# candrewlee14/zgml

Hardware: AMD Instinct MI355X
Metric: decode_tokens_per_sec (higher is better)
Workload: dtype f32; 1 GPU; SmolLM-135M Q4_0 greedy decode, batch 1, 1xMI355X (BASELINE configs[1]); weights=synthetic Q4_0 (int4 + f16 block scale / 32), tied f32 LM head, max_seq=2048, loop=device-resident (inputs in HBM), parallelism=none

## Files before the change

### zgml_amd/csrc/attention_decode.h

```cpp
#pragma once
#include "kernels.h"
#include "handoff_gen.h"
#include <hip/hip_fp16.h>
#include <math.h>

namespace zgml {
namespace {

typedef float f4v_t __attribute__((ext_vector_type(4)));
__device__ __forceinline__ float4 ldg4(const float* p) {
    const f4v_t v = *(const __attribute__((address_space(1))) f4v_t*)p;
    return make_float4(v.x, v.y, v.z, v.w);
}
__device__ __forceinline__ float ldg1(const float* p) { return *(const __attribute__((address_space(1))) float*)p; }
__device__ __forceinline__ uint32_t ldgu(const uint32_t* p) { return *(const __attribute__((address_space(1))) uint32_t*)p; }
__device__ __forceinline__ void stg4(float* p, float4 v) { *(__attribute__((address_space(1))) f4v_t*)p = f4v_t{v.x, v.y, v.z, v.w}; }
__device__ __forceinline__ void stg1(float* p, float v) { *(__attribute__((address_space(1))) float*)p = v; }
__device__ __forceinline__ void stgu(uint32_t* p, uint32_t v) { *(__attribute__((address_space(1))) uint32_t*)p = v; }

constexpr int kAttnBlock = 1024;
constexpr int kAttnUnroll = 4;

__device__ __forceinline__ float4 rope4(float4 own, float4 par, float4 c, float4 s, bool is_hi) {
    if (is_hi)
// ... 35 lines not shown
    if (LPK >= 2) v += __int_as_float(__builtin_amdgcn_mov_dpp(__float_as_int(v), 0xB1, 0xF, 0xF, true));
    if (LPK >= 4) v += __int_as_float(__builtin_amdgcn_mov_dpp(__float_as_int(v), 0x4E, 0xF, 0xF, true));
    if (LPK >= 8) v += __int_as_float(__builtin_amdgcn_mov_dpp(__float_as_int(v), 0x141, 0xF, 0xF, true));
    if (LPK >= 16) v += __int_as_float(__builtin_amdgcn_mov_dpp(__float_as_int(v), 0x140, 0xF, 0xF, true));
    if (LPK >= 32) v = xor16_sum(v);
    if (LPK >= 64) v = xor32_sum(v);
    return v;
}

struct SoftState {
    float m, l;
    float4 acc;
};
__device__ __forceinline__ void soft_merge(SoftState& s, float om, float ol, float4 oacc) {
    const float nm = fmaxf(s.m, om);
    const float a = s.m > -INFINITY ? expf(s.m - nm) : 0.0f, b = om > -INFINITY ? expf(om - nm) : 0.0f;
    s.l = s.l * a + ol * b;
    s.acc = make_float4(s.acc.x * a + oacc.x * b, s.acc.y * a + oacc.y * b, s.acc.z * a + oacc.z * b, s.acc.w * a + oacc.w * b);
    s.m = nm;
}

using gu64 = __attribute__((address_space(1))) unsigned long long;
using gu32 = __attribute__((address_space(1))) unsigned int;
__device__ __forceinline__ void split_put(float* p, float a, float b) {
    const unsigned long long v = (unsigned long long)__float_as_uint(a) | ((unsigned long long)__float_as_uint(b) << 32);
    __hip_atomic_store((gu64*)p, v, __ATOMIC_RELAXED, __HIP_MEMORY_SCOPE_AGENT);
}
__device__ __forceinline__ void split_get(const float* p, float& a, float& b) {
    const unsigned long long v = __hip_atomic_load((gu64*)p, __ATOMIC_RELAXED, __HIP_MEMORY_SCOPE_AGENT);
    a = __uint_as_float((uint32_t)v), b = __uint_as_float((uint32_t)(v >> 32));
}

template <int LPK>
__device__ __forceinline__ void slots_sum(SoftState& s) {
#pragma unroll
    for (int off = LPK; off < 16; off <<= 1) {
        s.l += __shfl_xor(s.l, off, 64);
        s.acc.x += __shfl_xor(s.acc.x, off, 64), s.acc.y += __shfl_xor(s.acc.y, off, 64);
        s.acc.z += __shfl_xor(s.acc.z, off, 64), s.acc.w += __shfl_xor(s.acc.w, off, 64);
    }
    if (LPK <= 16) s.l = xor16_sum(s.l), s.acc.x = xor16_sum(s.acc.x), s.acc.y = xor16_sum(s.acc.y), s.acc.z = xor16_sum(s.acc.z), s.acc.w = xor16_sum(s.acc.w);
    if (LPK <= 32) s.l = xor32_sum(s.l), s.acc.x = xor32_sum(s.acc.x), s.acc.y = xor32_sum(s.acc.y), s.acc.z = xor32_sum(s.acc.z), s.acc.w = xor32_sum(s.acc.w);
}
template <int LPK>
__device__ __forceinline__ void slots_merge(SoftState& s) {
    float M = s.m;
// ... 86 lines not shown
        __builtin_amdgcn_sched_barrier(0);
#endif
    }
}
template <int L, bool MAX>
__device__ __forceinline__ float slots_all(float v) {
    auto op = [](float a, float b) { return MAX ? fmaxf(a, b) : a + b; };
    if (L <= 1) v = op(v, __int_as_float(__builtin_amdgcn_mov_dpp(__float_as_int(v), 0x121, 0xF, 0xF, true)));
    if (L <= 2) v = op(v, __int_as_float(__builtin_amdgcn_mov_dpp(__float_as_int(v), 0x122, 0xF, 0xF, true)));
    if (L <= 4) v = op(v, __int_as_float(__builtin_amdgcn_mov_dpp(__float_as_int(v), 0x124, 0xF, 0xF, true)));
    if (L <= 8) v = op(v, __int_as_float(__builtin_amdgcn_mov_dpp(__float_as_int(v), 0x128, 0xF, 0xF, true)));
    if (L <= 16) v = MAX ? xor16_max(v) : xor16_sum(v);
    if (L <= 32) v = MAX ? xor32_max(v) : xor32_sum(v);
    return v;
}

struct DecodeHandoff {
    const unsigned long long* gran;
    uint32_t rel[3];
    uint32_t* gen;
    uint32_t n_heads;
    uint32_t* timeout;
    uint32_t poll_sleep;
};
__device__ __forceinline__ void handoff_idle(const DecodeHandoff* ho, uint32_t wg, uint32_t gen) { ho->gen[wg] = gen; }
__device__ __forceinline__ void handoff_idle(const CounterHandoff* ho, uint32_t wg, uint32_t) { for (int c = 0; c < 3; c++) ho->seen[3 * wg + c] += ho->need; }
__device__ __forceinline__ void handoff_done(const DecodeHandoff* ho, uint32_t wg, uint32_t gen, const uint32_t (&)[3]) { ho->gen[wg] = gen; }
__device__ __forceinline__ void handoff_done(const CounterHandoff* ho, uint32_t wg, uint32_t, const uint32_t (&t)[3]) { for (int c = 0; c < 3; c++) ho->seen[3 * wg + c] = t[c]; }
template <int LPK, bool KVQ, int BLOCK = kAttnBlock, typename HO = DecodeHandoff>
__device__ __forceinline__ void attention_decode_body(const AttnDecodeParams* __restrict__ params, float* split_buf, uint32_t* split_cnt,
                                                      uint32_t split_min_keys, const uint32_t hx, const uint32_t sp_in, const uint32_t n_sp, const HO* ho) {
    constexpr bool COUNTERS = std::is_same<HO, CounterHandoff>::value;
    constexpr int DH = 4 * LPK, HALF = DH / 2;
    constexpr bool Q16 = KVQ && ZGML_ATTN_KVQ16 != 0 && LPK >= 32;
    constexpr int LPKM = Q16 ? DH / 16 : LPK, KPW = 64 / LPKM, KPW4 = 64 / LPK, U = Q16 ? kAttnUnrollQ16 : kAttnUnroll;
    using Row = AttnRow<KVQ>;
    static_assert(sizeof(AttnDecodeParams) == 248, "the bulk fetch below covers exactly 62 dwords");
    AttnDecodeParams P;
    {
        typedef uint32_t u32x16_t __attribute__((ext_vector_type(16)));
        typedef uint32_t u32x8_t __attribute__((ext_vector_type(8)));
        typedef uint32_t u32x4_t __attribute__((ext_vector_type(4)));
        typedef uint32_t u32x2_t __attribute__((ext_vector_type(2)));
        u32x16_t ra, rb, rc;
        u32x8_t rd;
        u32x4_t re;
// ... 373 lines not shown
            ml[i] = *(const float2*)&part_ml[2 * wc];
            pa[i] = part_acc[wc * LPK + li];
        }
        M = fmaxf(M, __int_as_float(__builtin_amdgcn_mov_dpp(__float_as_int(M), 0xB1, 0xF, 0xF, true)));
        M = fmaxf(M, __int_as_float(__builtin_amdgcn_mov_dpp(__float_as_int(M), 0x4E, 0xF, 0xF, true)));
        M = fmaxf(M, __int_as_float(__builtin_amdgcn_mov_dpp(__float_as_int(M), 0x141, 0xF, 0xF, true)));
        M = fmaxf(M, __int_as_float(__builtin_amdgcn_mov_dpp(__float_as_int(M), 0x140, 0xF, 0xF, true)));
        M = __int_as_float(__builtin_amdgcn_readfirstlane(__float_as_int(M)));
        r = SoftState{M, 0.f, make_float4(0.f, 0.f, 0.f, 0.f)};
#pragma unroll
        for (int i = 0; i < NPS; i++) {
            const bool live = slot + i * KPW4 < NW && ml[i].x > -INFINITY;
            const float f = live ? expf(ml[i].x - M) : 0.0f;
            r.l += ml[i].y * f;
            r.acc.x += pa[i].x * f, r.acc.y += pa[i].y * f, r.acc.z += pa[i].z * f, r.acc.w += pa[i].w * f;
        }
        slots_sum<LPK>(r);
    } else {
        ATTN_STAMP(5);
        ATTN_STAMP(6);
    }
    {
        if (wait_qkv && lane == 0) handoff_done(ho, hx * n_sp + sp, gen, target);
        if (n_active > 1) {
            constexpr uint32_t REC = DH + 4;
            float* const head_buf = split_buf + (uint64_t)hx * n_sp * REC;
            float* const mine = head_buf + (uint64_t)sp * REC;
            if (lane < LPK) {
                if (lane == 0) split_put(mine, r.m, r.l);
                split_put(mine + 4 + 4 * lane, r.acc.x, r.acc.y);
                split_put(mine + 4 + 4 * lane + 2, r.acc.z, r.acc.w);
            }
            asm volatile("s_waitcnt vmcnt(0)" ::: "memory");
            uint32_t old = 0;
            if (lane == 0) old = __hip_atomic_fetch_add((gu32*)(split_cnt + hx), 1u, __ATOMIC_RELAXED, __HIP_MEMORY_SCOPE_AGENT);
            old = __shfl(old, 0, 64);
            if (old != n_active - 1) return;
            __builtin_amdgcn_fence(__ATOMIC_ACQUIRE, "wavefront");
            r = SoftState{-INFINITY, 0.f, make_float4(0.f, 0.f, 0.f, 0.f)};
            for (uint32_t c = slot; c < n_active; c += KPW4) {
                const float* rec = head_buf + (uint64_t)c * REC;
                float om, ol;
                float4 oa;
                split_get(rec, om, ol);
                split_get(rec + 4 + 4 * li, oa.x, oa.y);
                split_get(rec + 4 + 4 * li + 2, oa.z, oa.w);
// ... 28 lines not shown
```

### zgml_amd/csrc/kernels.h

```cpp
#pragma once

#include <hip/hip_runtime.h>
#include <stdint.h>
#include <stdlib.h>

#include "../../include/zgml_hip.h"
#include "sample.h"
#include "switches.h"

namespace zgml {

inline uint32_t device_cus() {
    static const uint32_t n = [] {
        int dev = 0, cus = 0;
        if (hipGetDevice(&dev) != hipSuccess || hipDeviceGetAttribute(&cus, hipDeviceAttributeMultiprocessorCount, dev) != hipSuccess || cus <= 0) cus = 256;
        return (uint32_t)cus;
    }();
    return n;
}

constexpr int kMaxFusedSteps = 8;

struct FusedStepDev {
    uint32_t op;
// ... 492 lines not shown
                  uint64_t* sc_bytes);
void launch_pack_qweight(hipStream_t s, const int8_t* raw_data, const float* raw_scales, const QWeightDev& out);
constexpr uint64_t kQmmScratchHead = 16384;
constexpr uint64_t kQmmCounterBytes = 4096;
uint64_t qmatmul_scratch_bytes(const QWeightDev& w, uint32_t M);
void launch_qmatmul(hipStream_t s, const QWeightDev& w, const QMatmulParams& p, float* scratch);
constexpr uint32_t kKonRowsMaxM = 8;
constexpr uint32_t kKonRowsRoutedM = 6;
bool launch_qmatvec_kon_rows(hipStream_t s, const QWeightDev& w, const QMatmulParams& p);
bool qmatmul_can_group(const QWeightDev& a, const QMatmulParams& pa, const QWeightDev& b, const QMatmulParams& pb);
uint32_t qmatmul_max_group();
void launch_qmatmul_group(hipStream_t s, const QWeightDev* w, const QMatmulParams* p, uint32_t n, float* scratch);
bool qmv_prenorm_ok(const QWeightDev& w, uint32_t K, uint64_t total_cols, uint32_t M);
bool qmv_pair_ok(const QWeightDev& w);
bool qmv_can_group(const QWeightDev& a, const QWeightDev& b);
uint32_t qmv_max_prologue_k(const QWeightDev& w);
void launch_qmatvec_fused(hipStream_t s, const QmvLaunch& L);
struct QkvHandoffBlock {
    unsigned long long* granules = nullptr;
    uint32_t *producer_gen = nullptr, *consumer_gen = nullptr;
    uint32_t* counters = nullptr;
    const uint32_t* idx = nullptr;
    uint32_t* seen = nullptr;
};
bool launch_qkv_attention(hipStream_t s, const QmvLaunch& L, const AttnDecodeParams* dev_params, uint32_t n_heads, uint32_t n_kv, uint32_t d_head,
                          const AttnSplit& sp, const QkvHandoffBlock& hb, uint32_t* timeout, bool kvq = false);
int qkv_attn_kon_census(hipStream_t s, uint32_t d_head, bool kvq, uint32_t grid);
int qkv_attn_kon_blocks_per_cu(uint32_t d_head, bool kvq);
void launch_synth_packed(hipStream_t s, const QWeightDev& w, uint32_t matrix_id);

struct KsVec {
    const float* base = nullptr;
    const float* parts = nullptr;
    uint32_t n_parts = 0;
    float* sum_dst = nullptr;
    float* add_dst = nullptr;
};
struct KsNormIn {
    KsVec x;
    const float* gamma = nullptr;
    float eps = 0.f;
    float* store_mid = nullptr;
    float* store_x = nullptr;
    uint32_t K = 0;
};
struct KsProjLaunch {
// ... 66 lines not shown
```

### zgml_amd/csrc/plan.hip

```cpp
#include "runtime_internal.h"

namespace {

float* buf_at(zgml_hip_program* p, uint16_t idx, uint64_t off) { return p->bufs[idx] + off; }

template <typename T>
const T* upload_params(zgml_hip_program* p, const std::vector<T>& v) {
    void* d = nullptr;
    if (hipMalloc(&d, v.size() * sizeof(T)) != hipSuccess) {
        p->ctx->fail("plan: parameter array allocation failed");
        return nullptr;
    }
    if (h2d_sync(p->ctx->stream, d, v.data(), v.size() * sizeof(T)) != hipSuccess) p->ctx->fail("plan: parameter array upload failed");
    p->param_blobs.push_back(d);
    return (const T*)d;
}

AttnSplit attn_split_for(zgml_hip_program* p, uint32_t n_heads, uint32_t d_head, uint32_t max_kv, int default_min_keys = 128) {
    const int want = sw().hip_attn_split;
    const int min_keys_env = sw().hip_attn_split_min_keys;
    AttnSplit sp;
    const int64_t min_keys = p->ctx->opt_attn_split_min_keys >= 0 ? p->ctx->opt_attn_split_min_keys : (min_keys_env >= 0 ? min_keys_env : default_min_keys);
    if (min_keys == 0 || want <= 1) return sp;
    sp.min_keys = (uint32_t)std::min<int64_t>(std::max<int64_t>(32, min_keys), 1 << 30);
// ... 501 lines not shown
}

void fuse_qkv_attention(zgml_hip_program* p) {
    if (!sw().hip_fuse_qkv_attn || p->ctx->fuse_qkv_off || !p->ctx->handoff_flag_dev) return;
    const uint64_t resident_cap = p->ctx->opt_fuse_resident_wgs >= 0 ? (uint64_t)p->ctx->opt_fuse_resident_wgs : (uint64_t)std::max(p->ctx->n_cu, 1);
    for (size_t i = 0; i + 1 < p->plan.size(); i++) {
        const auto qd = p->plan[i].qmv_desc;
        const auto ad = p->plan[i + 1].adec_desc;
        if (!qd || !ad) continue;
        const QmvLaunch& L = *qd;
        if (barrier_between_launches(p, i)) continue;
        const bool kon = L.parts[0].w.format == QW_Q4K && L.K > 2048;
        if (L.n_parts != 3 || (L.K > 2048 && !(kon && sw().hip_fuse_qkv_attn_kon)) || L.pro.kind == QMV_PRO_NONE || (ad->dh != 64 && ad->dh != 128) || L.trace) continue;
        if (kon && L.pro.kind != QMV_PRO_PRENORM) continue;
        const bool kvq = ad->kvq;
        bool ok = true;
        for (uint32_t t = 0; t < 3; t++) ok = ok && L.parts[t].n_epi == 0 && (L.parts[t].w.format == QW_Q4 || L.parts[t].w.format == QW_Q4K) && L.parts[t].w.scale_f16;
        const uint32_t nh = ad->nh, dh = ad->dh;
        ok = ok && (uint64_t)nh * dh == L.parts[0].w.N && L.parts[1].w.N == L.parts[2].w.N && L.parts[1].w.N % dh == 0;
        const uint32_t n_kv = ok ? (uint32_t)(L.parts[1].w.N / dh) : 0;
        ok = ok && n_kv != 0 && nh % n_kv == 0;
        std::vector<uint32_t> idx(3 * (size_t)nh);
        std::vector<char> head_seen(nh, 0);
        for (uint32_t r = 0; ok && r < nh; r++) {
            const AttnDecodeParams& a = ad->host[r];
            const ptrdiff_t qo = a.q_src - L.parts[0].dst, ko = a.k_src - L.parts[1].dst, vo = a.v_src - L.parts[2].dst;
            ok = qo >= 0 && qo % dh == 0 && (uint64_t)qo < (uint64_t)nh * dh && ko >= 0 && ko % dh == 0 && (uint64_t)ko < (uint64_t)n_kv * dh && vo == ko &&
                 a.kvq_block == (kvq ? 32u : 0u);
            if (!ok) break;
            const uint32_t h = (uint32_t)(qo / dh), kvh = (uint32_t)(ko / dh);
            ok = !head_seen[h] && kvh == h / (nh / n_kv);
            head_seen[h] = 1;
            idx[3 * r] = h, idx[3 * r + 1] = nh + kvh, idx[3 * r + 2] = nh + n_kv + kvh;
        }
        if (!ok) continue;
        uint32_t n_sp = ad->sp.splits ? ad->sp.splits : 1;
        uint64_t n_mv = 0;
        for (uint32_t t = 0; t < 3; t++) n_mv += L.parts[t].w.N / 16;
        uint64_t cap = resident_cap;
        if (kon && p->ctx->opt_fuse_resident_wgs < 0) {
            const int per_cu = qkv_attn_kon_blocks_per_cu(ad->dh, kvq);
            cap = per_cu > 0 ? (uint64_t)per_cu * (uint64_t)std::max(p->ctx->n_cu, 1) * (uint64_t)sw().hip_fuse_kon_cap_eighths / 8 : 0;
        }
        if (n_mv + nh > cap) continue;
        if (kon && p->ctx->opt_fuse_resident_wgs < 0 && (cap - n_mv) / nh < n_sp) continue;
        n_sp = (uint32_t)std::min<uint64_t>(n_sp, (cap - n_mv) / nh);
        for (uint32_t t = 0; kon && t < 3; t++) ok = ok && L.parts[t].w.format == QW_Q4K;
        if (!ok) continue;
        if (kon && p->ctx->opt_fuse_resident_wgs < 0) {
            const uint32_t grid = (uint32_t)(n_mv + (uint64_t)nh * n_sp);
            const uint64_t key = ((uint64_t)ad->dh << 40) | ((uint64_t)(kvq ? 1 : 0) << 32) | grid;
            auto it = p->ctx->census.find(key);
            if (it == p->ctx->census.end()) {
                const int r = sw().hip_fuse_census ? qkv_attn_kon_census(p->ctx->stream, ad->dh, kvq, grid) : -1;
                it = p->ctx->census.emplace(key, r).first;
                if (r == 0) fprintf(stderr, "[zgml_hip] the fused q/k/v + attention launch of %u workgroups is NOT co-resident on this device (census): two launches instead\n", grid);
            }
            if (it->second == 0) continue;
        }
        const size_t n_gran = ((size_t)nh + 2 * n_kv) * dh, n_cnt = 32 * ((size_t)nh + 2 * n_kv);
        const size_t bytes = kon ? (n_cnt + (size_t)nh * n_sp * 3 + 1 + idx.size()) * 4 : (n_gran * 8 + (n_mv + (size_t)nh * n_sp) * 4 + 15) / 16 * 16;
        void* block = nullptr;
        if (hipMalloc(&block, bytes) != hipSuccess) continue;
        if (memset_sync(p->ctx->stream, block, 0, bytes) != hipSuccess) {
            hipFree(block);
            continue;
        }
        p->fuse_owned.push_back(block);
        uint32_t* const timeout = p->ctx->handoff_flag_dev;
        QkvHandoffBlock hb;
        if (kon) {
            hb.counters = (uint32_t*)block, hb.seen = hb.counters + n_cnt;
            uint32_t* const idx_dev = hb.seen + (size_t)nh * n_sp * 3 + 1;
            if (h2d_sync(p->ctx->stream, idx_dev, idx.data(), idx.size() * 4) != hipSuccess) continue;
            hb.idx = idx_dev;
        } else {
            hb.granules = (unsigned long long*)block;
            hb.producer_gen = (uint32_t*)(hb.granules + n_gran), hb.consumer_gen = hb.producer_gen + n_mv;
        }
        const AttnDecodeParams* d = ad->dev;
        AttnSplit sp = ad->sp;
        sp.splits = n_sp;
        const uint32_t n_ops = p->plan[i].n_ops + p->plan[i + 1].n_ops, lo = std::min(p->plan[i].op_lo, p->plan[i + 1].op_lo),
                       hi = std::max(p->plan[i].op_hi, p->plan[i + 1].op_hi);
        Launch F{ZGML_DOP_QMATMUL, n_ops, lo, hi, [=](hipStream_t s) {
                     if (!launch_qkv_attention(s, L, d, nh, n_kv, dh, sp, hb, timeout, kvq)) {
                         launch_qmatvec_fused(s, L);
                         launch_attention_decode_batch(s, d, nh, dh, sp, kvq);
                     }
                 }};
        p->plan[i] = std::move(F);
        p->plan.erase(p->plan.begin() + (ptrdiff_t)i + 1);
    }
}

void fuse_ksplit(zgml_hip_program* p) {
    p->has_deferred = false;
    if (!p->ksplit || p->ksplit_off || !p->barriers.empty()) return;
    auto overlap = [](const float* a, size_t na, const float* b, size_t nb) { return a && b && a < b + nb && b < a + na; };
    auto residual_epi = [](const QmvPart& pt) {
        return pt.n_epi == 1 && pt.epi[0].op == ZGML_OP_ADD && pt.epi[0].operand && pt.epi[0].operand != pt.dst && pt.epi[0].store && pt.epi[0].store != pt.dst;
// ... 1121 lines not shown
```

### zgml_amd/csrc/qmatvec.hip

```cpp
#include "qmv_common.h"
#include "attention_decode.h"

#include <hip/hip_fp16.h>
#include <math.h>
#include <stdlib.h>
#include <string.h>

#include <type_traits>
#include <utility>

namespace zgml {

namespace {



struct QMVPartDev {
    const uint4* qs;
    const void* sc;
    float* out;
    uint32_t NB2;
    uint32_t block_begin;
    uint32_t out_rs;
    uint32_t n_epi;
// ... 110 lines not shown
                                             bool have_pre0 = false) {
    const float raw = v;
#pragma unroll
    for (uint32_t e = 0; e < (uint32_t)kMaxEpiSteps; e++) {
        if (e >= part.n_epi) break;
        const QmvEpiStep st = part.epi[e];
        if (st.op == ZGML_OP_ADD) {
            const float o = st.operand == out_row ? raw : (e == 0 && have_pre0 ? pre0 : st.operand[n]);
            v = st.swapped ? o + v : v + o;
        } else if (st.op == ZGML_OP_MUL) {
            const float o = st.operand == out_row ? raw : (e == 0 && have_pre0 ? pre0 : st.operand[n]);
            v = st.swapped ? o * v : v * o;
        } else {
            v = epi_unary(st.op, v);
        }
        if (st.store) st.store[n] = v;
    }
}

struct QmvPublish {
    unsigned long long* gran;
    uint32_t* gen;
    uint32_t drop;
};
struct QmvCountPublish {
    uint32_t* cnt;
    uint32_t base[3];
    uint32_t groups_shift;
    uint32_t drop;
};

struct KonTail {
    float post;
    bool norm;
    float eps;
    uint32_t K;
    float a_s, b_s;
    uint32_t k0, slice;
    bool has_pro;
    bool prenorm;
    float pp[4];
    bool inv_known = false;
    float inv_pre = 1.0f;
};
__device__ __forceinline__ float prenorm_factor(const float (&pp)[4], uint32_t K, float eps) {
    const float ss = rows_sum4(row16_sum((pp[0] + pp[1]) + (pp[2] + pp[3])));
    return 1.0f / sqrtf(ss / (float)K + eps);
}
__device__ __forceinline__ float kon_factor_and_slices(const KonTail& kt, const QMVArgs& a, const float* red, uint32_t n_waves, uint32_t lane) {
    const uint32_t col = lane & 15;
    float inv = 1.0f;
    if (kt.inv_known) {
        inv = kt.inv_pre;
    } else if (kt.prenorm) {
        float s4 = (kt.pp[0] + kt.pp[1]) + (kt.pp[2] + kt.pp[3]);
        for (uint32_t j = lane + 256; j < a.pro.n_ssq; j += 64) s4 += a.pro.ssq[j];
        const float ss = rows_sum4(row16_sum(s4));
        inv = 1.0f / sqrtf(ss / (float)kt.K + kt.eps);
    } else if (kt.norm) {
        const float sv = red[kMaxWaves * 16 + min(col, n_waves - 1)];
        const float ss = row16_sum(col < n_waves ? sv : 0.f);
        inv = 1.0f / sqrtf(ss / (float)kt.K + kt.eps);
    }
    if (kt.has_pro && lane < 16) {
        const QmvPrologue& pr = a.pro;
        if (kt.slice <= 16) {
            const uint32_t k = kt.k0 + lane;
            if (lane < kt.slice && k < kt.K) {
                const float mid = kt.norm ? kt.a_s * inv : kt.a_s;
                if (kt.norm && pr.store_mid) pr.store_mid[k] = mid;
                if (pr.store_x) pr.store_x[k] = mid * kt.b_s;
            }
        } else {
            for (uint32_t k = kt.k0 + lane; k < min(kt.k0 + kt.slice, kt.K); k += 16) {
                const float mid = kt.norm ? pr.a[k] * inv : pr.a[k];
                if (kt.norm && pr.store_mid) pr.store_mid[k] = mid;
                if (pr.store_x) pr.store_x[k] = mid * pr.b[k];
            }
        }
    }
    return inv;
}
template <bool GROUPED, bool KON = false, typename PUB = QmvPublish>
__device__ __forceinline__ void reduce_store(float acc, float* red, const QMVArgs& a, uint32_t pi, float* out0, uint32_t g, uint32_t m,
                                             float pre0, bool have_pre0, uint32_t n_waves, const PUB* pub = nullptr, const KonTail* kon = nullptr,
                                             float pre_g = 0.f, uint32_t pub_cg = 0, uint32_t pub_gen = 0) {
    const uint32_t lane = threadIdx.x & 63, w = __builtin_amdgcn_readfirstlane(threadIdx.x >> 6);
    if (!KON) {
        acc = rows_sum4(acc);
        if (lane < 16) red[w * 16 + lane] = acc;
    }
    uint32_t kind = kEpiGeneric;
    float ones = 0.f;
    if (GROUPED) {
        kind = pi == 1 ? a.parts[1].epi_kind : pi == 2 ? a.parts[2].epi_kind : pi == 3 ? a.parts[3].epi_kind : a.parts[0].epi_kind;
        if (kind == kEpiSilu && w == 0) {
            const float* const ones_p = pi == 1 ? a.parts[1].epi[2].operand : pi == 2 ? a.parts[2].epi[2].operand : pi == 3 ? a.parts[3].epi[2].operand : a.parts[0].epi[2].operand;
            ones = ones_p[g * 16 + (lane & 15)];
        }
    }
    __syncthreads();
    if (w != 0) return;
    const uint32_t r = lane >> 4, col = lane & 15;
    float part[4];
#pragma unroll
    for (uint32_t j = 0; j < 4; j++) part[j] = red[min(r + 4 * j, n_waves - 1) * 16 + col];
    float v = 0.f;
#pragma unroll
    for (uint32_t j = 0; j < 4; j++) v += r + 4 * j < n_waves ? part[j] : 0.f;
    v = rows_sum4(v);
    if (KON) v *= kon->post * kon_factor_and_slices(*kon, a, red, n_waves, lane);
    if (!KON && kon) v *= kon_factor_and_slices(*kon, a, red, n_waves, lane);
    if (lane < 16) {
        const uint32_t n = g * 16 + threadIdx.x;
        float* out = out0;
        if (GROUPED) out = pi == 1 ? a.parts[1].out : pi == 2 ? a.parts[2].out : pi == 3 ? a.parts[3].out : out;
        float* out_row = out;
        if (m) {
            uint32_t out_rs = a.parts[0].out_rs;
            if (GROUPED) out_rs = pi == 1 ? a.parts[1].out_rs : pi == 2 ? a.parts[2].out_rs : pi == 3 ? a.parts[3].out_rs : out_rs;
            out_row = out + (uint64_t)m * out_rs;
        }
        constexpr bool COUNTERS = std::is_same<PUB, QmvCountPublish>::value;
        if constexpr (COUNTERS) {
            if (pub)
                __hip_atomic_store((__attribute__((address_space(1))) float*)out_row + n, v, __ATOMIC_RELAXED, __HIP_MEMORY_SCOPE_AGENT);
            else
                out_row[n] = v;
        } else {
            if (pub && !(pub->drop && pub_cg == 0))
                __hip_atomic_store((gu64*)pub->gran + (pub_cg * 16 + lane), handoff_granule(__float_as_uint(v), pub_gen), __ATOMIC_RELAXED, __HIP_MEMORY_SCOPE_AGENT);
            out_row[n] = v;
        }
        if (GROUPED && kind == kEpiSilu) {
            if (pi == 0)
                run_epilogue_silu(a.parts[0], n, v, ones);
            else if (pi == 1)
                run_epilogue_silu(a.parts[1], n, v, ones);
            else if (pi == 2)
                run_epilogue_silu(a.parts[2], n, v, ones);
            else
                run_epilogue_silu(a.parts[3], n, v, ones);
        } else if (!GROUPED && have_pre0 && a.parts[0].epi_kind == kEpiResidual) {
            const float h = v + pre0;
            a.parts[0].epi[0].store[n] = h;
            if (a.next.xg_out) {
                a.next.xg_out[n] = h * pre_g;
                const float sq = row16_sum(h * h);
                if (lane == 0) a.next.ssq_out[g] = sq;
            }
        } else if (!GROUPED && have_pre0 && a.parts[0].epi_kind == kEpiMulVec) {
            a.parts[0].epi[0].store[n] = v * pre0;
        } else if (!GROUPED || pi == 0)
            run_epilogue(a.parts[0], n, v, out_row, pre0, !GROUPED && have_pre0);
        else if (pi == 1)
            run_epilogue(a.parts[1], n, v, out_row);
        else if (pi == 2)
            run_epilogue(a.parts[2], n, v, out_row);
        else
            run_epilogue(a.parts[3], n, v, out_row);
    }
    if constexpr (std::is_same<PUB, QmvCountPublish>::value) {
        if (pub) {
#if defined(__HIP_DEVICE_COMPILE__)
            asm volatile("s_waitcnt vmcnt(0)" ::: "memory");
#endif
            if (lane == 0 && !(pub->drop && pi == 0 && g == 0))
                __hip_atomic_fetch_add((__attribute__((address_space(1))) uint32_t*)pub->cnt + 32 * (pub->base[pi < 3 ? pi : 2] + (g >> pub->groups_shift)), 1u,
                                       __ATOMIC_RELAXED, __HIP_MEMORY_SCOPE_AGENT);
        }
    } else {
        if (pub && lane == 0) pub->gen[pub_cg] = pub_gen;
    }
}



struct XDirect {
    const float* a;
    const float* b;
    float* store_x;
    float* store_mid;
    uint32_t K;
    float inv;
    bool norm;
    __device__ __forceinline__ float pro_value(float av, float bv, uint32_t k, bool live) const {
        float v = av;
        if (norm) {
            v = av * inv;
            if (store_mid && live) store_mid[k] = v;
        }
        v = v * bv;
        if (store_x && live) store_x[k] = v;
        return v;
    }
// ... 549 lines not shown
#undef QMV_STAMP
}

template <int DEPTH, int PROM, bool GROUPED, bool XV, bool NT>
__global__ void __launch_bounds__(1024) qmatvec_kon_kernel(QMV_HEAD_PARAMS, QMVArgs a) {
    qmatvec_kon_body<DEPTH, PROM, GROUPED, XV, NT>(qs0, sc0, out0, xa_base, xb_base, in_rs, K, nb2_0_flags, nb2_12, a, blockIdx.x, gridDim.x, nullptr);
}
template <int DEPTH, int PROM, bool NT>
__global__ void __launch_bounds__(512, 4) qmatvec_kon_pair_kernel(QMV_HEAD_PARAMS, QMVArgs a) {
    qmatvec_kon_body<DEPTH, PROM, true, true, NT, true>(qs0, sc0, out0, xa_base, xb_base, in_rs, K, nb2_0_flags, nb2_12, a, blockIdx.x, gridDim.x, nullptr);
}

struct QkvAttnArgs {
    const AttnDecodeParams* params;
    float* split_buf;
    uint32_t* split_cnt;
    uint32_t split_min_keys, n_mv, n_sp;
    uint32_t kvq;
    QmvPublish pub;
    DecodeHandoff ho;
    QmvCountPublish cpub;
    CounterHandoff cho;
    uint32_t* census;
};
template <typename ST, bool Q4, int LPK, bool KVQ, int PROM = 1>
__global__ void __launch_bounds__(1024) qkv_attn_kernel(QMV_HEAD_PARAMS, QMVArgs a, QkvAttnArgs f) {
    constexpr int DEPTH = 1;
    if (blockIdx.x < f.n_mv) {
        const uint32_t n_waves = ((nb2_0_flags >> 20) & 0xFu) + 1;
        if (threadIdx.x >= n_waves * 64) return;
        qmatvec_body<ST, false, DEPTH, Q4, PROM, true, true, false>(qs0, sc0, out0, xa_base, xb_base, in_rs, K, nb2_0_flags, nb2_12, a, blockIdx.x, &f.pub);
    } else {
        const uint32_t b = blockIdx.x - f.n_mv, n_heads = f.ho.n_heads;
        attention_decode_body<LPK, KVQ>(f.params, f.split_buf, f.split_cnt, f.split_min_keys, b % n_heads, b / n_heads, f.n_sp, &f.ho);
    }
}

template <int LPK, int DEPTH, int PROM, bool NT, bool KVQ, bool CENSUS = false>
__global__ void __launch_bounds__(256, 4) qkv_attn_kon_kernel(QMV_HEAD_PARAMS, QMVArgs a, QkvAttnArgs f) {
    if (CENSUS && f.census) {
        if (threadIdx.x == 0) {
            using gu32c = __attribute__((address_space(1))) uint32_t;
            __hip_atomic_fetch_add((gu32c*)f.census, 1u, __ATOMIC_RELAXED, __HIP_MEMORY_SCOPE_AGENT);
            const uint64_t t0 = __builtin_amdgcn_s_memrealtime();
            while (__hip_atomic_load((gu32c*)f.census, __ATOMIC_RELAXED, __HIP_MEMORY_SCOPE_AGENT) < gridDim.x) {
                if (__builtin_amdgcn_s_memrealtime() - t0 > 20000u) {
                    __hip_atomic_store((gu32c*)f.census + 1, 1u, __ATOMIC_RELAXED, __HIP_MEMORY_SCOPE_AGENT);
                    break;
                }
                __builtin_amdgcn_s_sleep(8);
            }
        }
        return;
    }
    if (blockIdx.x < f.n_mv) {
        qmatvec_kon_body<DEPTH, PROM, true, true, NT>(qs0, sc0, out0, xa_base, xb_base, in_rs, K, nb2_0_flags, nb2_12, a, blockIdx.x, f.n_mv, &f.cpub);
// ... 425 lines not shown
            return false;
        }
        const KernelFn pf = prenorm ? (depth_sel == 0 ? qmatvec_pair_kernel<1, 2> : depth_sel == 1 ? qmatvec_pair_kernel<2, 2> : qmatvec_pair_kernel<4, 2>)
                                    : (depth_sel == 0 ? qmatvec_pair_kernel<1, 0> : depth_sel == 1 ? qmatvec_pair_kernel<2, 0> : qmatvec_pair_kernel<4, 0>);
        const size_t lds2 = ((size_t)(2 * kMaxWaves + 1) * 16) * sizeof(float);
        hipLaunchKernelGGL(pf, dim3(a.parts[0].NB2), dim3(waves * 64), lds2, s, a.parts[0].qs, a.parts[0].sc, a.parts[0].out, head_xa, head_xb, a.in_rs, a.K,
                           head_flags(a, waves, true, false, late), nb2_12, a);
        return true;
    }
    if (fused) {
        if (!(xd && (pro || prenorm) && grp && !nt && q4 && w0.scale_f16 && contig && M == 1 && a.n_parts == 3 && (d_head == 64 || d_head == 128) && fused->ho.gran)) return false;
        QkvAttnArgs f = *fused;
        f.n_mv = total_blocks;
        const bool fused_kvq = f.kvq != 0;
        if (depth_sel != 0) return false;
        using FusedFn = void (*)(const uint4*, const void*, float*, const float*, const float*, uint32_t, uint32_t, uint32_t, uint32_t, QMVArgs, QkvAttnArgs);
        FusedFn ff = nullptr;
        if (d_head == 64)
            ff = prenorm ? (fused_kvq ? qkv_attn_kernel<__half, true, 16, true, 2> : qkv_attn_kernel<__half, true, 16, false, 2>)
                         : (fused_kvq ? qkv_attn_kernel<__half, true, 16, true> : qkv_attn_kernel<__half, true, 16, false>);
        else
            ff = prenorm ? (fused_kvq ? qkv_attn_kernel<__half, true, 32, true, 2> : qkv_attn_kernel<__half, true, 32, false, 2>)
                         : (fused_kvq ? qkv_attn_kernel<__half, true, 32, true> : qkv_attn_kernel<__half, true, 32, false>);
        hipLaunchKernelGGL(ff, dim3(total_blocks + extra_blocks), dim3(1024), lds, s, a.parts[0].qs, a.parts[0].sc, a.parts[0].out, head_xa, head_xb, a.in_rs, a.K,
                           head_flags(a, waves, true, rmsnorm, late), nb2_12, a, f);
        return true;
    }
    hipLaunchKernelGGL(fn, grid, dim3(waves * 64), lds, s, a.parts[0].qs, a.parts[0].sc, a.parts[0].out, head_xa, head_xb, a.in_rs, a.K,
                       head_flags(a, waves, contig, rmsnorm, late), nb2_12, a);
    return true;
}

}

uint32_t qmv_max_prologue_k(const QWeightDev& w) { return w.format == QW_Q4K ? UINT32_MAX : kMaxWaves * 64 * 4 * kXRegs; }

void launch_qmatvec_rows(hipStream_t s, const QWeightDev& w, const QMatmulParams& p, bool xvec) {
    QMVArgs a{};
    a.n_parts = 1;
    a.parts[0].qs = (const uint4*)w.qs;
    a.parts[0].sc = w.sc;
    a.parts[0].out = p.dst;
    a.parts[0].NB2 = p.N / 16;
    a.parts[0].block_begin = 0;
    a.parts[0].out_rs = p.dst_rs;
    a.parts[0].n_epi = 0;
    a.pro.kind = QMV_PRO_NONE;
// ... 55 lines not shown
    build_qmv_args(L, a, blocks, xvec);
    return launch_packed(s, a, L.parts[0].w, blocks, 1, xvec, fused, extra_blocks, d_head);
}

void launch_qmatvec_fused(hipStream_t s, const QmvLaunch& L) { launch_qmv(s, L, nullptr, 0, 0); }

bool launch_qkv_attention(hipStream_t s, const QmvLaunch& L, const AttnDecodeParams* dev_params, uint32_t n_heads, uint32_t n_kv, uint32_t d_head,
                          const AttnSplit& sp, const QkvHandoffBlock& hb, uint32_t* timeout, bool kvq) {
    if (L.n_parts != 3) return false;
    QkvAttnArgs f{};
    f.kvq = kvq ? 1 : 0;
    f.params = dev_params, f.split_buf = sp.buf, f.split_cnt = sp.cnt, f.split_min_keys = sp.min_keys;
    f.n_sp = sp.splits ? sp.splits : 1;
    const uint32_t drop = sw().hip_debug_drop_publish ? 1u : 0u;
    if (hb.counters) {
        uint32_t shift = 0;
        while ((16u << shift) < d_head) shift++;
        f.cpub = QmvCountPublish{hb.counters, {0, n_heads, n_heads + n_kv}, shift, drop};
        f.cho = CounterHandoff{hb.counters, hb.seen, hb.idx, n_heads, d_head / 16, timeout, (uint32_t)sw().hip_handoff_sleep};
        return launch_qmv(s, L, &f, n_heads * f.n_sp, d_head);
    }
    if (!hb.granules) return false;
    unsigned long long* const granules = hb.granules;
    f.pub = QmvPublish{granules, hb.producer_gen, drop};
    const uint32_t first[3] = {0, n_heads * d_head, (n_heads + n_kv) * d_head};
    f.ho = DecodeHandoff{granules, {0, 0, 0}, hb.consumer_gen, n_heads, timeout, (uint32_t)sw().hip_handoff_sleep};
    for (int c = 0; c < 3; c++) f.ho.rel[c] = 8u * first[c] - 2u * (uint32_t)(uintptr_t)L.parts[c].dst;
    return launch_qmv(s, L, &f, n_heads * f.n_sp, d_head);
}

int qkv_attn_kon_census(hipStream_t s, uint32_t d_head, bool kvq, uint32_t grid) {
    using Fn = void (*)(const uint4*, const void*, float*, const float*, const float*, uint32_t, uint32_t, uint32_t, uint32_t, QMVArgs, QkvAttnArgs);
    const Fn census = d_head == 64 ? (kvq ? (Fn)qkv_attn_kon_kernel<16, 4, 2, true, true, true> : (Fn)qkv_attn_kon_kernel<16, 4, 2, true, false, true>)
                                   : (kvq ? (Fn)qkv_attn_kon_kernel<32, 4, 2, true, true, true> : (Fn)qkv_attn_kon_kernel<32, 4, 2, true, false, true>);
    const Fn product = d_head == 64 ? (kvq ? (Fn)qkv_attn_kon_kernel<16, 4, 2, true, true> : (Fn)qkv_attn_kon_kernel<16, 4, 2, true, false>)
                                    : (kvq ? (Fn)qkv_attn_kon_kernel<32, 4, 2, true, true> : (Fn)qkv_attn_kon_kernel<32, 4, 2, true, false>);
    hipFuncAttributes fa{}, fb{};
    if (hipFuncGetAttributes(&fa, (const void*)census) != hipSuccess || hipFuncGetAttributes(&fb, (const void*)product) != hipSuccess) return -1;
    if (fa.numRegs < fb.numRegs || fa.sharedSizeBytes != fb.sharedSizeBytes) return -1;
    uint32_t* blk = nullptr;
    if (hipMalloc((void**)&blk, 8) != hipSuccess) return -1;
    int result = -1;
    uint32_t host[2] = {0, 1};
    if (hipMemsetAsync(blk, 0, 8, s) == hipSuccess) {
        QMVArgs a{};
        QkvAttnArgs f{};
        f.census = blk;
        const size_t lds = ((size_t)kMaxWaves * 16 + kMaxWaves) * sizeof(float);
        hipLaunchKernelGGL(census, dim3(grid), dim3(256), lds, s, (const uint4*)nullptr, (const void*)nullptr, (float*)nullptr, (const float*)nullptr, (const float*)nullptr, 0u, 0u, 0u,
                           0u, a, f);
// ... 24 lines not shown
```

### zgml_amd/csrc/qmv_common.h

```cpp
#pragma once
#include "kernels.h"

#include <hip/hip_fp16.h>
#include <hip/hip_runtime.h>
#include <stdint.h>

namespace zgml {

void launch_qmatvec_rows(hipStream_t s, const QWeightDev& w, const QMatmulParams& p, bool xvec);

namespace {

constexpr int kBlock = 256;
constexpr int kMaxWaves = 16;

#define ZGML_SDWA "dst_sel:DWORD dst_unused:UNUSED_PAD src0_sel:BYTE_"

__device__ __forceinline__ float to_f32(__half h) { return __half2float(h); }
__device__ __forceinline__ float to_f32(float f) { return f; }

template <bool XVEC>
__device__ __forceinline__ float4 load_x4(const float* x, uint32_t i, uint32_t K) {
    if (XVEC) return *(const float4*)(x + (i < K ? i : 0));
    const uint32_t last = K - 1;
    return make_float4(x[min(i, last)], x[min(i + 1, last)], x[min(i + 2, last)], x[min(i + 3, last)]);
}

__device__ __forceinline__ float4 zero_tail(float4 v, uint32_t i, uint32_t K) {
    return make_float4(i < K ? v.x : 0.f, i + 1 < K ? v.y : 0.f, i + 2 < K ? v.z : 0.f, i + 3 < K ? v.w : 0.f);
}

__device__ __forceinline__ uint32_t column_group(uint32_t b, uint32_t NB2) {
    const uint32_t full = NB2 & ~15u;
    if (b >= full) return b;
    const uint32_t j = (b >> 4) * 8 + (b & 7), half = (b >> 3) & 1;
    return 2 * j + half;
}

template <bool NT>
__device__ __forceinline__ uint4 wload(const uint4* p) {
    if (NT) {
        typedef unsigned int u4v __attribute__((ext_vector_type(4)));
        const u4v v = __builtin_nontemporal_load((const u4v*)p);
        return make_uint4(v.x, v.y, v.z, v.w);
    }
    return *p;
}

#define ZGML_DPP(i) " row_newbcast:%" #i " row_mask:0xf bank_mask:0xf\n\t"

template <int BASE>
__device__ __forceinline__ void q4_dword(float& accA, float& accB, uint32_t w, float t) {
    float c0, c1, c2, c3;
    uint32_t h;
    asm("v_cvt_off_f32_i4_sdwa %2, %7 " ZGML_SDWA "0\n\t"
        "v_cvt_off_f32_i4_sdwa %3, %7 " ZGML_SDWA "1\n\t"
        "v_cvt_off_f32_i4_sdwa %4, %7 " ZGML_SDWA "2\n\t"
        "v_cvt_off_f32_i4_sdwa %5, %7 " ZGML_SDWA "3\n\t"
        "v_lshrrev_b32 %6, 4, %7\n\t"
// ... 119 lines not shown
```

### zgml_amd/csrc/runtime.hip

```cpp
#include "runtime_internal.h"

namespace zgml_rt {
std::string g_create_error;
}

namespace {


void fill_caps(zgml_capabilities* c) {
    memset(c, 0, sizeof(*c));
    c->compiled_programs = 1;
    c->host_visible_program_memory = 0;
    c->dense_matmul_f32 = 1;
    c->dense_matmul_f16 = 1;
    c->qmatmul = 1;
    c->fused_elementwise = 1;
    c->max_fused_elementwise_steps_has = 1;
    c->max_fused_elementwise_steps = kMaxFusedSteps;
    c->f16_weight_promotion = 1;
    c->dynamic_program_refresh = 1;
    c->prefill_attention = 1;
    c->decode_attention = 1;
    c->quantized_kv = 1;
    c->command_buffer_execution = 1;
// ... 1260 lines not shown
}

void shard_peer_release(zgml_hip_program* p);
void zgml_hip_free_program(zgml_hip_ctx* ctx, zgml_hip_program* p) {
    if (!p) return;
    if (ctx) {
        hipSetDevice(ctx->device);
        hipStreamSynchronize(ctx->stream);
    }
    if (ctx && !ctx->handoff_ok("free_program")) fprintf(stderr, "[zgml_hip] ERROR: %s\n", ctx->err.c_str());
    for (void* d : p->fuse_owned) hipFree(d);
    if (!p->attn_traces.empty()) {
        fprintf(stderr, "[zgml_hip] attention trace (ns since previous launch's end | start->params | ->dyn | ->rope | ->scores | ->max | ->pv | ->end)\n");
        unsigned long long prev_end = 0;
        for (size_t i = 0; i < p->attn_traces.size(); i++) {
            const unsigned long long* t = p->attn_traces[i];
            fprintf(stderr, "  L%02zu gap %6lld |", i, prev_end ? (long long)(t[0] - prev_end) * 10 : -1);
            for (int k = 1; k < 8; k++) fprintf(stderr, " %5lld", (long long)(t[k] - t[k - 1]) * 10);
            fprintf(stderr, "\n");
            prev_end = t[7];
        }
        for (auto* t : p->attn_traces) hipHostFree(t);
    }
    if (!p->ks_traces.empty()) {
        fprintf(stderr, "[zgml_hip] K-split launches, workgroup 0, ns between stamps (gap = since the previous launch's last stamp); ks-proj / ks-mlp: start | loads issued | "
                        "parts summed | vector whole | x staged | FMAs | barrier | folded (mlp: + SiLU) | (mlp: barrier | down partial); ks-attn-o: start | record | loads issued | attention | merged | partial O\n");
        unsigned long long prev_end = 0;
        for (const auto& k : p->ks_traces) {
            int last = 0;
            for (int j = 0; j < 16; j++)
                if (k.t[j]) last = j;
            fprintf(stderr, "  %-10s gap %6lld |", k.what, prev_end ? (long long)(k.t[0] - prev_end) * 10 : -1);
            for (int j = 1; j <= last; j++) fprintf(stderr, " %5lld", k.t[j] ? (long long)(k.t[j] - k.t[j - 1]) * 10 : -1);
            fprintf(stderr, " | span %5lld\n", (long long)(k.t[last] - k.t[0]) * 10);
            if (k.t[16]) {
                fprintf(stderr, "      last wave: start %+5lld |", (long long)(k.t[16] - k.t[0]) * 10);
                for (int j = 1; j <= last && j < 12; j++) fprintf(stderr, " %5lld", k.t[16 + j] ? (long long)(k.t[16 + j] - k.t[16 + j - 1]) * 10 : -1);
                fprintf(stderr, "\n");
            }
            prev_end = k.t[last];
        }
        for (auto& k : p->ks_traces) hipHostFree(k.t);
    }
    if (!p->qmv_traces.empty()) {
        fprintf(stderr, "[zgml_hip] mat-vec trace, workgroup 0 (ns: gap since previous mat-vec end | ->loads issued | ->x arrived(+sumsq) | ->x staged | ->streamed | ->reduced+epilogue)"
                        " || K-on-lanes launches also: LAST workgroup, start after workgroup 0's start | ->loads issued | ->streamed | ->end; launch span = first start -> last end\n");
// ... 146 lines not shown
```

### zgml_amd/csrc/runtime_internal.h

```cpp
#pragma once
#include <hip/hip_runtime.h>

#include <algorithm>
#include <chrono>
#include <cstdio>
#include <cstdlib>
#include <cstring>
#include <functional>
#include <map>
#include <memory>
#include <string>
#include <vector>

#include "dev_block.h"
#include "kernels.h"
#include "schedule.h"

using namespace zgml;

namespace zgml_rt {

extern std::string g_create_error;

struct SplitHook {
// ... 141 lines not shown
    }

    void fail(const std::string& what) {
        if (err.empty()) err = what;
    }
    bool check(hipError_t e, const char* what) {
        if (e == hipSuccess) return true;
        fail(std::string(what) + ": " + hipGetErrorString(e));
        return false;
    }
};

struct zgml_resident;
struct zgml_hip_program {
    zgml_hip_ctx* ctx = nullptr;
    std::vector<zgml_device_op> ops;
    std::vector<uint32_t> dyn_ops;
    std::vector<std::vector<zgml_fused_step>> steps;
    std::vector<uint64_t> sizes;
    std::vector<float*> bufs;
    void* arena = nullptr;
    std::vector<QWeightDev> qweights;
    std::vector<unsigned long long*> attn_traces;
    struct QmvTrace {
        unsigned long long* t;
        uint32_t parts, pro, K, N;
    };
    std::vector<QmvTrace> qmv_traces;
    struct KsTrace {
        unsigned long long* t;
        const char* what;
    };
    std::vector<KsTrace> ks_traces;
    float* zero_word = nullptr;
    float* split_buf = nullptr;
    uint32_t* split_cnt = nullptr;
    uint64_t split_buf_floats = 0, split_cnt_words = 0;
    bool f16_stream_nt = false;
    std::vector<void*> f16_weights;
    std::vector<void*> owned;
    uint64_t fuse_epoch = 0;
    std::vector<void*> fuse_owned;
    std::vector<char> hoist_op;
    std::vector<char> hoist_guard;
    bool hoist_ok = true;
    bool ksplit = false;
// ... 87 lines not shown
```

Before: 1755 tokens/s.

## Colocate fused QKV producer and attention consumer workgroups on the same XCD

Remaps block indices in the fused q/k/v + attention kernel so each KV group's producer column-groups and its consuming attention heads land on the same XCD (blockIdx mod 8), aiming to keep the handoff granules in a shared L2 and avoid cross-die polling latency. It also moves the prenorm slice writes after the granule publish so consumers see outputs earlier. Adds XCC-ID tracing under ZGML_TRACE for verification. The remap adds per-block index arithmetic and depends on hardware round-robin dispatch of workgroups to XCDs.

```diff
diff --git a/zgml_amd/csrc/attention_decode.h b/zgml_amd/csrc/attention_decode.h
--- a/zgml_amd/csrc/attention_decode.h
+++ b/zgml_amd/csrc/attention_decode.h
@@ -81,6 +81,15 @@
 
 using gu64 = __attribute__((address_space(1))) unsigned long long;
 using gu32 = __attribute__((address_space(1))) unsigned int;
+#ifdef ZGML_TRACE
+__device__ __forceinline__ uint32_t xcc_id() {
+    uint32_t x = 0;
+#if defined(__HIP_DEVICE_COMPILE__)
+    asm volatile("s_getreg_b32 %0, hwreg(HW_REG_XCC_ID)" : "=s"(x));
+#endif
+    return x & 0xFu;
+}
+#endif
 __device__ __forceinline__ void split_put(float* p, float a, float b) {
     const unsigned long long v = (unsigned long long)__float_as_uint(a) | ((unsigned long long)__float_as_uint(b) << 32);
     __hip_atomic_store((gu64*)p, v, __ATOMIC_RELAXED, __HIP_MEMORY_SCOPE_AGENT);
@@ -213,6 +222,7 @@
     uint32_t n_heads;
     uint32_t* timeout;
     uint32_t poll_sleep;
+    uint32_t* xcc;
 };
 __device__ __forceinline__ void handoff_idle(const DecodeHandoff* ho, uint32_t wg, uint32_t gen) { ho->gen[wg] = gen; }
 __device__ __forceinline__ void handoff_idle(const CounterHandoff* ho, uint32_t wg, uint32_t) { for (int c = 0; c < 3; c++) ho->seen[3 * wg + c] += ho->need; }
@@ -632,6 +642,11 @@
     }
     {
         if (wait_qkv && lane == 0) handoff_done(ho, hx * n_sp + sp, gen, target);
+#ifdef ZGML_TRACE
+        if constexpr (!COUNTERS) {
+            if (wait_qkv && ho->xcc && lane == 0) ho->xcc[hx * n_sp + sp] = 1 + xcc_id();
+        }
+#endif
         if (n_active > 1) {
             constexpr uint32_t REC = DH + 4;
             float* const head_buf = split_buf + (uint64_t)hx * n_sp * REC;
diff --git a/zgml_amd/csrc/kernels.h b/zgml_amd/csrc/kernels.h
--- a/zgml_amd/csrc/kernels.h
+++ b/zgml_amd/csrc/kernels.h
@@ -538,6 +538,8 @@
     uint32_t* counters = nullptr;
     const uint32_t* idx = nullptr;
     uint32_t* seen = nullptr;
+    bool group_order = false;
+    uint32_t* xcc_trace = nullptr;
 };
 bool launch_qkv_attention(hipStream_t s, const QmvLaunch& L, const AttnDecodeParams* dev_params, uint32_t n_heads, uint32_t n_kv, uint32_t d_head,
                           const AttnSplit& sp, const QkvHandoffBlock& hb, uint32_t* timeout, bool kvq = false);
diff --git a/zgml_amd/csrc/plan.hip b/zgml_amd/csrc/plan.hip
--- a/zgml_amd/csrc/plan.hip
+++ b/zgml_amd/csrc/plan.hip
@@ -547,6 +547,7 @@
         ok = ok && n_kv != 0 && nh % n_kv == 0;
         std::vector<uint32_t> idx(3 * (size_t)nh);
         std::vector<char> head_seen(nh, 0);
+        bool group_order = true;
         for (uint32_t r = 0; ok && r < nh; r++) {
             const AttnDecodeParams& a = ad->host[r];
             const ptrdiff_t qo = a.q_src - L.parts[0].dst, ko = a.k_src - L.parts[1].dst, vo = a.v_src - L.parts[2].dst;
@@ -556,6 +557,7 @@
             const uint32_t h = (uint32_t)(qo / dh), kvh = (uint32_t)(ko / dh);
             ok = !head_seen[h] && kvh == h / (nh / n_kv);
             head_seen[h] = 1;
+            group_order = group_order && kvh == r / (nh / n_kv);
             idx[3 * r] = h, idx[3 * r + 1] = nh + kvh, idx[3 * r + 2] = nh + n_kv + kvh;
         }
         if (!ok) continue;
@@ -602,6 +604,10 @@
         } else {
             hb.granules = (unsigned long long*)block;
             hb.producer_gen = (uint32_t*)(hb.granules + n_gran), hb.consumer_gen = hb.producer_gen + n_mv;
+            hb.group_order = group_order;
+            const size_t n_wg = (size_t)n_mv + (size_t)nh * n_sp;
+            if (sw().hip_attn_trace && (hb.xcc_trace = (uint32_t*)mapped_trace((n_wg + 1) / 2)))
+                p->xcc_traces.push_back({hb.xcc_trace, (uint32_t)n_mv, nh, n_kv, dh, n_sp});
         }
         const AttnDecodeParams* d = ad->dev;
         AttnSplit sp = ad->sp;
diff --git a/zgml_amd/csrc/qkv_colocate.h b/zgml_amd/csrc/qkv_colocate.h
--- /dev/null
+++ b/zgml_amd/csrc/qkv_colocate.h
@@ -0,0 +1,60 @@
+#pragma once
+#include <stdint.h>
+
+#if defined(__HIPCC__) || defined(__CUDACC__)
+#define ZGML_COLOCATE_HD __host__ __device__
+#else
+#define ZGML_COLOCATE_HD
+#endif
+
+namespace zgml {
+
+struct QkvColocate {
+    uint32_t on;
+    uint32_t n_kv;
+    uint32_t pk;
+    uint32_t hpg;
+};
+ZGML_COLOCATE_HD inline uint32_t qkv_colocate_pack(const QkvColocate& c) { return c.on ? 0x80000000u | (c.hpg << 16) | (c.pk << 8) | c.n_kv : 0u; }
+ZGML_COLOCATE_HD inline QkvColocate qkv_colocate_unpack(uint32_t w) { return QkvColocate{w >> 31, w & 0xFFu, (w >> 8) & 0xFFu, (w >> 16) & 0x7FFFu}; }
+
+ZGML_COLOCATE_HD inline uint32_t qkv_colocate_groups_on(uint32_t label, uint32_t n_kv) { return label < n_kv ? (n_kv - label + 7) >> 3 : 0; }
+ZGML_COLOCATE_HD inline uint32_t qkv_colocate_ids_on(uint32_t label, uint32_t grid) { return grid > label ? (grid - label + 7) >> 3 : 0; }
+
+inline QkvColocate qkv_colocate_plan(uint32_t n_heads, uint32_t n_kv, uint32_t d_head, uint32_t n_sp) {
+    QkvColocate c{};
+    if (!n_heads || !n_kv || n_heads % n_kv || !d_head || d_head % 16 || !n_sp) return c;
+    const uint32_t hpg = n_heads / n_kv, pk = d_head / 16, per_group = (hpg + 2) * pk + hpg;
+    if (n_kv > 255 || pk > 255 || hpg > 32767) return c;
+    const unsigned long long grid = (unsigned long long)n_kv * (hpg + 2) * pk + (unsigned long long)n_heads * n_sp;
+    if (grid >= (1ull << 31)) return c;
+    for (uint32_t l = 0; l < 8; l++)
+        if ((unsigned long long)qkv_colocate_groups_on(l, n_kv) * per_group > qkv_colocate_ids_on(l, (uint32_t)grid)) return c;
+    c.on = 1, c.n_kv = n_kv, c.pk = pk, c.hpg = hpg;
+    return c;
+}
+
+ZGML_COLOCATE_HD inline uint32_t qkv_colocate_role(const QkvColocate& c, uint32_t b, uint32_t n_mv, uint32_t n_heads, uint32_t n_sp) {
+    if (!c.on) return b;
+    const uint32_t label = b & 7, pq = c.hpg * c.pk, p = pq + 2 * c.pk, groups = qkv_colocate_groups_on(label, c.n_kv);
+    const uint32_t n_pro = groups * p, n_con = groups * c.hpg;
+    uint32_t t = b >> 3, j = label;
+    if (t < n_pro) {
+        while (t >= p) t -= p, j += 8;
+        if (t < pq) return j * pq + t;
+        if (t < pq + c.pk) return c.n_kv * pq + j * c.pk + (t - pq);
+        return c.n_kv * (pq + c.pk) + j * c.pk + (t - pq - c.pk);
+    }
+    t -= n_pro;
+    if (t < n_con) {
+        while (t >= c.hpg) t -= c.hpg, j += 8;
+        return n_mv + j * c.hpg + t;
+    }
+    const uint32_t grid = n_mv + n_heads * n_sp;
+    uint32_t rank = t - n_con;
+    for (uint32_t l = 0; l < 7; l++)
+        if (l < label) rank += qkv_colocate_ids_on(l, grid) - qkv_colocate_groups_on(l, c.n_kv) * (p + c.hpg);
+    return n_mv + n_heads + rank;
+}
+
+}
diff --git a/zgml_amd/csrc/qmatvec.hip b/zgml_amd/csrc/qmatvec.hip
--- a/zgml_amd/csrc/qmatvec.hip
+++ b/zgml_amd/csrc/qmatvec.hip
@@ -1,5 +1,6 @@
 #include "qmv_common.h"
 #include "attention_decode.h"
+#include "qkv_colocate.h"
 
 #include <hip/hip_fp16.h>
 #include <math.h>
@@ -156,6 +157,7 @@
     unsigned long long* gran;
     uint32_t* gen;
     uint32_t drop;
+    uint32_t* xcc;
 };
 struct QmvCountPublish {
     uint32_t* cnt;
@@ -181,7 +183,7 @@
     const float ss = rows_sum4(row16_sum((pp[0] + pp[1]) + (pp[2] + pp[3])));
     return 1.0f / sqrtf(ss / (float)K + eps);
 }
-__device__ __forceinline__ float kon_factor_and_slices(const KonTail& kt, const QMVArgs& a, const float* red, uint32_t n_waves, uint32_t lane) {
+__device__ __forceinline__ float kon_factor(const KonTail& kt, const QMVArgs& a, const float* red, uint32_t n_waves, uint32_t lane) {
     const uint32_t col = lane & 15;
     float inv = 1.0f;
     if (kt.inv_known) {
@@ -196,6 +198,9 @@
         const float ss = row16_sum(col < n_waves ? sv : 0.f);
         inv = 1.0f / sqrtf(ss / (float)kt.K + kt.eps);
     }
+    return inv;
+}
+__device__ __forceinline__ void kon_slices(const KonTail& kt, const QMVArgs& a, float inv, uint32_t lane) {
     if (kt.has_pro && lane < 16) {
         const QmvPrologue& pr = a.pro;
         if (kt.slice <= 16) {
@@ -213,6 +218,10 @@
             }
         }
     }
+}
+__device__ __forceinline__ float kon_factor_and_slices(const KonTail& kt, const QMVArgs& a, const float* red, uint32_t n_waves, uint32_t lane) {
+    const float inv = kon_factor(kt, a, red, n_waves, lane);
+    kon_slices(kt, a, inv, lane);
     return inv;
 }
 template <bool GROUPED, bool KON = false, typename PUB = QmvPublish>
@@ -244,7 +253,9 @@
     for (uint32_t j = 0; j < 4; j++) v += r + 4 * j < n_waves ? part[j] : 0.f;
     v = rows_sum4(v);
     if (KON) v *= kon->post * kon_factor_and_slices(*kon, a, red, n_waves, lane);
-    if (!KON && kon) v *= kon_factor_and_slices(*kon, a, red, n_waves, lane);
+    float pn_inv = 1.0f;
+    const bool slices_last = !KON && kon && pub && !std::is_same<PUB, QmvCountPublish>::value;
+    if (!KON && kon) v *= pn_inv = slices_last ? kon_factor(*kon, a, red, n_waves, lane) : kon_factor_and_slices(*kon, a, red, n_waves, lane);
     if (lane < 16) {
         const uint32_t n = g * 16 + threadIdx.x;
         float* out = out0;
@@ -265,6 +276,7 @@
             if (pub && !(pub->drop && pub_cg == 0))
                 __hip_atomic_store((gu64*)pub->gran + (pub_cg * 16 + lane), handoff_granule(__float_as_uint(v), pub_gen), __ATOMIC_RELAXED, __HIP_MEMORY_SCOPE_AGENT);
             out_row[n] = v;
+            if (slices_last) kon_slices(*kon, a, pn_inv, lane);
         }
         if (GROUPED && kind == kEpiSilu) {
             if (pi == 0)
@@ -305,6 +317,9 @@
         }
     } else {
         if (pub && lane == 0) pub->gen[pub_cg] = pub_gen;
+#ifdef ZGML_TRACE
+        if (pub && pub->xcc && lane == 0) pub->xcc[pub_cg] = 1 + xcc_id();
+#endif
     }
 }
 
@@ -900,16 +915,26 @@
     QmvCountPublish cpub;
     CounterHandoff cho;
     uint32_t* census;
+    uint32_t colocate;
 };
 template <typename ST, bool Q4, int LPK, bool KVQ, int PROM = 1>
 __global__ void __launch_bounds__(1024) qkv_attn_kernel(QMV_HEAD_PARAMS, QMVArgs a, QkvAttnArgs f) {
     constexpr int DEPTH = 1;
-    if (blockIdx.x < f.n_mv) {
+    const uint32_t NB2_0 = nb2_0_flags & 0xFFFFFu, NB2_1 = nb2_12 & 0xFFFFu, NB2_2 = nb2_12 >> 16, n_mv = NB2_0 + NB2_1 + NB2_2;
+    const QkvColocate co = qkv_colocate_unpack(in_rs);
+    const uint32_t role = qkv_colocate_role(co, blockIdx.x, n_mv, f.ho.n_heads, f.n_sp);
+    if (role < n_mv) {
         const uint32_t n_waves = ((nb2_0_flags >> 20) & 0xFu) + 1;
         if (threadIdx.x >= n_waves * 64) return;
-        qmatvec_body<ST, false, DEPTH, Q4, PROM, true, true, false>(qs0, sc0, out0, xa_base, xb_base, in_rs, K, nb2_0_flags, nb2_12, a, blockIdx.x, &f.pub);
+        uint32_t bx = role;
+        if (co.on) {
+            const uint32_t pi = role < NB2_0 ? 0u : role < NB2_0 + NB2_1 ? 1u : 2u;
+            const uint32_t first = pi == 0 ? 0u : pi == 1 ? NB2_0 : NB2_0 + NB2_1, nb2 = pi == 0 ? NB2_0 : pi == 1 ? NB2_1 : NB2_2;
+            bx = first + column_group_block(role - first, nb2);
+        }
+        qmatvec_body<ST, false, DEPTH, Q4, PROM, true, true, false>(qs0, sc0, out0, xa_base, xb_base, K, K, nb2_0_flags, nb2_12, a, bx, &f.pub);
     } else {
-        const uint32_t b = blockIdx.x - f.n_mv, n_heads = f.ho.n_heads;
+        const uint32_t b = role - n_mv, n_heads = f.ho.n_heads;
         attention_decode_body<LPK, KVQ>(f.params, f.split_buf, f.split_cnt, f.split_min_keys, b % n_heads, b / n_heads, f.n_sp, &f.ho);
     }
 }
@@ -1381,7 +1406,7 @@
         else
             ff = prenorm ? (fused_kvq ? qkv_attn_kernel<__half, true, 32, true, 2> : qkv_attn_kernel<__half, true, 32, false, 2>)
                          : (fused_kvq ? qkv_attn_kernel<__half, true, 32, true> : qkv_attn_kernel<__half, true, 32, false>);
-        hipLaunchKernelGGL(ff, dim3(total_blocks + extra_blocks), dim3(1024), lds, s, a.parts[0].qs, a.parts[0].sc, a.parts[0].out, head_xa, head_xb, a.in_rs, a.K,
+        hipLaunchKernelGGL(ff, dim3(total_blocks + extra_blocks), dim3(1024), lds, s, a.parts[0].qs, a.parts[0].sc, a.parts[0].out, head_xa, head_xb, f.colocate, a.K,
                            head_flags(a, waves, true, rmsnorm, late), nb2_12, a, f);
         return true;
     }
@@ -1483,10 +1508,12 @@
     }
     if (!hb.granules) return false;
     unsigned long long* const granules = hb.granules;
-    f.pub = QmvPublish{granules, hb.producer_gen, drop};
+    f.pub = QmvPublish{granules, hb.producer_gen, drop, hb.xcc_trace};
     const uint32_t first[3] = {0, n_heads * d_head, (n_heads + n_kv) * d_head};
-    f.ho = DecodeHandoff{granules, {0, 0, 0}, hb.consumer_gen, n_heads, timeout, (uint32_t)sw().hip_handoff_sleep};
+    f.ho = DecodeHandoff{granules, {0, 0, 0}, hb.consumer_gen, n_heads, timeout, (uint32_t)sw().hip_handoff_sleep,
+                         hb.xcc_trace ? hb.xcc_trace + (n_heads + 2 * n_kv) * (d_head / 16) : nullptr};
     for (int c = 0; c < 3; c++) f.ho.rel[c] = 8u * first[c] - 2u * (uint32_t)(uintptr_t)L.parts[c].dst;
+    if (hb.group_order) f.colocate = qkv_colocate_pack(qkv_colocate_plan(n_heads, n_kv, d_head, f.n_sp));
     return launch_qmv(s, L, &f, n_heads * f.n_sp, d_head);
 }
 
diff --git a/zgml_amd/csrc/qmv_common.h b/zgml_amd/csrc/qmv_common.h
--- a/zgml_amd/csrc/qmv_common.h
+++ b/zgml_amd/csrc/qmv_common.h
@@ -35,6 +35,12 @@
     if (b >= full) return b;
     const uint32_t j = (b >> 4) * 8 + (b & 7), half = (b >> 3) & 1;
     return 2 * j + half;
+}
+__device__ __forceinline__ uint32_t column_group_block(uint32_t g, uint32_t NB2) {
+    const uint32_t full = NB2 & ~15u;
+    if (g >= full) return g;
+    const uint32_t j = g >> 1, half = g & 1;
+    return (j >> 3) * 16 + half * 8 + (j & 7);
 }
 
 template <bool NT>
diff --git a/zgml_amd/csrc/runtime.hip b/zgml_amd/csrc/runtime.hip
--- a/zgml_amd/csrc/runtime.hip
+++ b/zgml_amd/csrc/runtime.hip
@@ -1306,6 +1306,26 @@
         }
         for (auto* t : p->attn_traces) hipHostFree(t);
     }
+    if (!p->xcc_traces.empty()) {
+        uint64_t pairs0 = 0, same0 = 0, pairs_n = 0, same_n = 0;
+        for (const auto& x : p->xcc_traces) {
+            const uint32_t pk = x.d_head / 16, hpg = x.n_heads / x.n_kv, nq = x.n_heads * pk, nk = x.n_kv * pk;
+            for (uint32_t r = 0; r < x.n_heads; r++)
+                for (uint32_t sp = 0; sp < x.n_sp; sp++) {
+                    const uint32_t c = x.w[x.n_mv + r * x.n_sp + sp];
+                    if (!c) continue;
+                    for (uint32_t i = 0; i < 3 * pk; i++) {
+                        const uint32_t part = i / pk, g = i % pk, cg = part == 0 ? r * pk + g : nq + (part - 1) * nk + (r / hpg) * pk + g;
+                        if (!x.w[cg]) continue;
+                        (sp ? pairs_n : pairs0)++;
+                        if (x.w[cg] == c) (sp ? same_n : same0)++;
+                    }
+                }
+        }
+        fprintf(stderr, "[zgml_hip] fused q/k/v + attention, %zu launches: producer / consumer pairs on one XCD: split 0 %llu of %llu, splits >= 1 %llu of %llu\n",
+                p->xcc_traces.size(), (unsigned long long)same0, (unsigned long long)pairs0, (unsigned long long)same_n, (unsigned long long)pairs_n);
+        for (const auto& x : p->xcc_traces) hipHostFree(x.w);
+    }
     if (!p->ks_traces.empty()) {
         fprintf(stderr, "[zgml_hip] K-split launches, workgroup 0, ns between stamps (gap = since the previous launch's last stamp); ks-proj / ks-mlp: start | loads issued | "
                         "parts summed | vector whole | x staged | FMAs | barrier | folded (mlp: + SiLU) | (mlp: barrier | down partial); ks-attn-o: start | record | loads issued | attention | merged | partial O\n");
diff --git a/zgml_amd/csrc/runtime_internal.h b/zgml_amd/csrc/runtime_internal.h
--- a/zgml_amd/csrc/runtime_internal.h
+++ b/zgml_amd/csrc/runtime_internal.h
@@ -187,6 +187,11 @@
     void* arena = nullptr;
     std::vector<QWeightDev> qweights;
     std::vector<unsigned long long*> attn_traces;
+    struct XccTrace {
+        uint32_t* w;
+        uint32_t n_mv, n_heads, n_kv, d_head, n_sp;
+    };
+    std::vector<XccTrace> xcc_traces;
     struct QmvTrace {
         unsigned long long* t;
         uint32_t parts, pro, K, N;
```

Result: faster. 1780 tokens/s (median of 6 runs) (+1.4%).
